# FengDushuo/BBBP-Multi-Modal-Deep-Ensemble-Framework

Measured on AMD Instinct MI355X. Metric: molecules/sec fwd+bwd (3-branch ensemble, B=512), higher is better.
Workload: dtype f32; 1 GPU; MixedInputModel F=167 (MACCS) + 3x128x128 image, 6-layer encoder + 2-stage CNN + fusion + BN head; forward + MSE + backward + fused AdamW, train mode (dropout 0.1); global_batch=512, per_gpu_batch=512, parallelism=dp1, input=device-resident

## Files before the change

bbbp-multi-modal-deep-ensemble-framework_amd/csrc/common.h:

```cpp
#pragma once
#include <hip/hip_runtime.h>
#include <stdint.h>
#include <stdio.h>
#include <string.h>

typedef float f32x16 __attribute__((ext_vector_type(16)));
typedef float f32x4 __attribute__((ext_vector_type(4)));
typedef float f32x2 __attribute__((ext_vector_type(2)));

#define BBBP_OK 0
#define BBBP_ERR_ARG 1
#define BBBP_ERR_HIP 2
#define BBBP_ERR_WORKSPACE 3

void bbbp_set_error(const char* fmt, ...);

#define BBBP_CHECK_ARG(cond, ...)                 \
    do {                                          \
        if (!(cond)) {                            \
            bbbp_set_error(__VA_ARGS__);          \
            return BBBP_ERR_ARG;                  \
        }                                         \
    } while (0)

#define BBBP_CHECK_HIP(expr)                                                            \
    do {                                                                                \
        hipError_t _e = (expr);                                                         \
        if (_e != hipSuccess) {                                                         \
            bbbp_set_error("%s failed: %s (%s:%d)", #expr, hipGetErrorString(_e), __FILE__, __LINE__); \
            return BBBP_ERR_HIP;                                                        \
        }                                                                               \
    } while (0)

#define BBBP_CHECK_LAUNCH() BBBP_CHECK_HIP(hipGetLastError())

static inline int cdiv(int a, int b) { return (a + b - 1) / b; }
static inline size_t align_up(size_t x, size_t a) { return (x + a - 1) / a * a; }

int bbbp_num_cus();
static inline int persistent_grid(int want, int nmb, int nwork) {
    int grid = want;
    if (grid >= 8 * nmb) grid -= grid % (8 * nmb);
    if (grid > nwork) grid = nwork - nwork % nmb;
    return grid < nmb ? nmb : grid;
}
int bbbp_ensure_dyn_lds(const void* kernel, size_t bytes);
template <class P>
int launch_lds(void (*kernel)(P), dim3 grid, int threads, size_t lds, hipStream_t st, const P& p) {
    if (int rc = bbbp_ensure_dyn_lds(reinterpret_cast<const void*>(kernel), lds)) return rc;
    void* args[] = {const_cast<P*>(&p)};
    BBBP_CHECK_HIP(hipLaunchKernel(reinterpret_cast<const void*>(kernel), grid, dim3(threads), args, lds, st));
    return BBBP_OK;
}
const char* bbbp_env(const char* name);
int bbbp_env_int(const char* name, int dflt);
static inline int clampi(int v, int lo, int hi) { return v < lo ? lo : (v > hi ? hi : v); }
struct Knob {
    const char* env; int dflt; int (*norm)(int);
    int v = -1;
    int get() { if (v < 0) v = norm(bbbp_env_int(env, dflt)); return v; }
    int set(int x) { const int prev = get(); v = norm(x); return prev; }
};
static inline int knob_bool(int v) { return v != 0; }

extern thread_local int g_bbbp_reserved_cus;
extern thread_local size_t g_bbbp_small_lds_pad;
struct ConvPrefs {
    int conv1_fwd_f32 = 0;
    int conv1_fwd_per_cu = 0;
    int conv2_fwd_pipe = 0;
    int wgrad_beside_encoder = 0;
};
enum ConvMaskBit {
    CONV_WINO_FWD = 1, CONV_WINO_DGRAD = 2,
    CONV_B3_FWD = 4, CONV_B3_DGRAD = 8, CONV_B3_WGRAD = 16,
    CONV_B3_C1_WGRAD = 32, CONV_B3_C1_FWD = 64,
    CONV_B3_WGRAD_SPARSE = 128, CONV_B3_WGRAD_SPARSE4 = 256,
    CONV_MASK_ALL = 511
};
enum class ConvForm { F32Direct, Winograd, SplitBf16, SplitBf16Pipe, Conv1SplitBf16, Conv1SplitBf16Pipe, WgradDense, WgradSparse8, WgradSparse4 };
int conv3x3_relu_pool_fwd(hipStream_t st, const float* x, const float* w, const float* bias, float* y, uint8_t* mask, int B, int cin, int cout,
                          int H, int W, void* workspace, size_t workspace_bytes, const ConvPrefs& prefs);
int conv3x3_relu_pool_bwd_weight(hipStream_t st, const float* x, const float* gy, const uint8_t* gmask, float* dw, float* dbias, int B, int cin,
                                 int cout, int H, int W, void* workspace, size_t workspace_bytes, const ConvPrefs& prefs);
extern thread_local int g_bbbp_wino_side_cus;
int bbbp_head_forward_fused(hipStream_t st, const float* comb, const float* const* fw1, const float* const* fb1,
                            const float* const* fw2, const float* const* fb2, const float* w0, const float* b0, const float* gamma,
                            const float* beta, float* running_mean, float* running_var, const float* w3, const float* b3,
                            const float* w5, const float* b5, const float* w7, const float* b7, float* hid, float* attn, float* fused,
                            float* h, float* hb, float* bn_mean, float* bn_rstd, float* h2, float* h3, float* out, float* partial,
                            int B, int training, int concat);
int bbbp_head_backward_fused(hipStream_t st, const float* dout, const float* comb, const float* hid, const float* attn, const float* h,
                             const float* h2, const float* h3, const float* bn_mean, const float* bn_rstd, const float* gamma,
                             const float* const* fw1, const float* const* fw2, const float* w0, const float* w3, const float* w5,
                             const float* w7, float* dh3, float* dh2, float* dhb, float* dh, float* dlogit, float* dpre, float* dcomb,
                             float* dgamma, float* dbeta, float* partial, int B, int training);
struct bbbp_enc_row_fwd_args {
    const float* ctx; const float* xin;
    const float *wo, *bo, *g1, *be1, *w1, *b1, *w2, *b2, *g2, *be2;
    const float *wn, *bn; float* outn; int nn, ldn, actn;
    float *z1, *y1, *hff, *z2, *y2, *mean1, *rstd1, *mean2, *rstd2;
    int B, F, DFF; float p; uint64_t seed1, seed2, seed3;
};
struct bbbp_enc_row_bwd_args {
    const float* dqkv_up; const float* win_up; const float* dz1_up; float* dyout;
    const float *z2, *mean2, *rstd2, *g2, *w2, *hff, *w1, *z1, *mean1, *rstd1, *g1, *wo;
    float *dz2, *dff, *dhff, *dy1, *dz1, *dsa, *dctx;
    int B, F, DFF; float p; uint64_t seed1, seed3;
};
bool bbbp_enc_rows_supported(int F, int nhead, int dff);
int bbbp_enc_row_fwd(hipStream_t st, const bbbp_enc_row_fwd_args* a);
int bbbp_enc_row_bwd(hipStream_t st, const bbbp_enc_row_bwd_args* a);
int bbbp_ln_param_grad_multi(hipStream_t st, int n, const float* const* dy, const float* const* z, const float* const* mean,
                             const float* const* rstd, float* const* dgamma, float* const* dbeta, int rows, int cols);
bool bbbp_attn_small_supported(int B, int nhead, int head_dim);
bool bbbp_attn_wide_supported(int B, int nhead, int head_dim);
size_t bbbp_attn_small_keep_bytes(int B, int nhead, int head_dim);
int bbbp_attn_small_fwd(hipStream_t st, const float* qkv, float* ctx, float* lse, int B, int F, int nhead, float scale, float p, uint64_t seed,
                        uint8_t* keep = nullptr);
int bbbp_attn_small_bwd(hipStream_t st, const float* qkv, const float* ctx, const float* lse, const float* dctx, float* dqkv, int B, int F,
                        int nhead, float scale, float p, uint64_t seed, const uint8_t* keep = nullptr);
constexpr size_t BBBP_CONV_MIN_LDS = 120 * 1024;
int bbbp_wino_conv2_fwd(hipStream_t st, const float* x, const float* w, const float* bias, float* y, uint8_t* mask, int B,
                        float* workspace);
int bbbp_wino_conv2_dgrad(hipStream_t st, const float* gy, const uint8_t* gmask, const float* w, float* dx, int B, float* workspace);
int bbbp_wino_last_clock(unsigned long long* shader_cycles, unsigned long long* ticks_100mhz);
bool bbbp_b3_conv_supported(int cin, int cout, int hw);
size_t bbbp_b3_workspace_bytes(int cin, int cout);
int bbbp_b3_conv_fwd(hipStream_t st, const float* x, const float* w, const float* bias, float* y, uint8_t* mask, int B, int cin, int cout, void* workspace,
                     ConvForm form, int per_cu, bool probe);
int bbbp_b3_conv_dgrad(hipStream_t st, const float* gy, const uint8_t* gmask, const float* w, float* dx, int B, int cin, int cout, void* workspace,
                       ConvForm form, int per_cu, bool probe);
int bbbp_b3_conv2_wgrad(hipStream_t st, const float* x, const float* gy, const uint8_t* mask, float* slab, float* bslab, int B, int grid, ConvForm form,
                        int cin_total, int cout_total, int groups, int map);
int bbbp_b3_last_clock(unsigned long long* shader_cycles, unsigned long long* ticks_100mhz);
size_t bbbp_b3_conv1_fwd_workspace_bytes();
int bbbp_b3_conv1_fwd(hipStream_t st, const float* x, const float* w, const float* bias, float* y, uint8_t* mask, int B, void* workspace,
                      ConvForm form, int per_cu);
int bbbp_b3_conv1_wgrad(hipStream_t st, const float* x, const float* gy, const uint8_t* mask, float* slab, float* bslab, int B, int grid);
int bbbp_wino_last_phases(unsigned long long* phases4);
int bbbp_param_wait(hipStream_t st, const void* ptr);
bool bbbp_param_pending_elsewhere(const void* ptr);
bool bbbp_layernorm_linear_preferred(int M, int N, int K);
bool bbbp_outproj_fold_supported(int F, int nhead, int layers);
size_t bbbp_outproj_fold_floats(int F, int which);
int bbbp_outproj_fold(hipStream_t st, int layers, int F, const float* const* win, const float* const* bin, const float* const* wo,
                      const float* const* bo, float* const* wf, float* const* bf, float* const* wvt);
int bbbp_outproj_unfold(hipStream_t st, int F, int B, const float* tdw, const float* tdb, const float* wo, const float* wvt, const float* dz,
                        int lddz, float* g_outw, float* g_outb, float* g_inw_v, float* g_inb_v);

__device__ __forceinline__ int xcd_adjacent(int w, int n) { return (n & 7) ? w : (w & 7) * (n >> 3) + (w >> 3); }

__device__ __forceinline__ f32x16 mfma32(float a, float b, f32x16 c) {
    return __builtin_amdgcn_mfma_f32_32x32x2f32(a, b, c, 0, 0, 0);
}
__device__ __forceinline__ int mfma_row(int r, int lane) { return (r & 3) + 8 * (r >> 2) + 4 * (lane >> 5); }

typedef __bf16 bf16x8 __attribute__((ext_vector_type(8)));
typedef __bf16 bf16x2 __attribute__((ext_vector_type(2)));
typedef float f32x2v __attribute__((ext_vector_type(2)));
typedef uint32_t u32x4 __attribute__((ext_vector_type(4)));
typedef uint32_t u32x2 __attribute__((ext_vector_type(2)));
__device__ __forceinline__ void split2(float a, float b, uint32_t& hi, uint32_t& mid, uint32_t& lo) {
    f32x2v v = {a, b};
    bf16x2 h = __builtin_convertvector(v, bf16x2);
    hi = __builtin_bit_cast(uint32_t, h);
    f32x2v hf = {__builtin_bit_cast(float, hi << 16), __builtin_bit_cast(float, hi & 0xffff0000u)};
    v = v - hf;
    bf16x2 m = __builtin_convertvector(v, bf16x2);
    mid = __builtin_bit_cast(uint32_t, m);
    f32x2v mf = {__builtin_bit_cast(float, mid << 16), __builtin_bit_cast(float, mid & 0xffff0000u)};
    v = v - mf;
    bf16x2 l = __builtin_convertvector(v, bf16x2);
    lo = __builtin_bit_cast(uint32_t, l);
}

__device__ __forceinline__ uint4 philox4(uint64_t seed, uint64_t ctr) {
    uint32_t k0 = (uint32_t)seed, k1 = (uint32_t)(seed >> 32);
    uint32_t c0 = (uint32_t)ctr, c1 = (uint32_t)(ctr >> 32), c2 = 0x9E3779B9u, c3 = 0xBB67AE85u;
#pragma unroll
    for (int i = 0; i < 10; ++i) {
        uint64_t p0 = (uint64_t)0xD2511F53u * c0;
        uint64_t p1 = (uint64_t)0xCD9E8D57u * c2;
        uint32_t n0 = (uint32_t)(p1 >> 32) ^ c1 ^ k0;
        uint32_t n1 = (uint32_t)p1;
        uint32_t n2 = (uint32_t)(p0 >> 32) ^ c3 ^ k1;
        uint32_t n3 = (uint32_t)p0;
        c0 = n0; c1 = n1; c2 = n2; c3 = n3;
        k0 += 0x9E3779B9u; k1 += 0xBB67AE85u;
    }
    return make_uint4(c0, c1, c2, c3);
}
extern thread_local const unsigned long long* g_bbbp_seed_base;
__device__ __forceinline__ uint64_t effective_seed(uint64_t seed, const unsigned long long* base) {
    return base ? (uint64_t)(*base) * 0x9E3779B97F4A7C15ull + seed : seed;
}
__device__ __forceinline__ float dropout_scale(uint64_t seed, uint64_t idx, float p, float inv_keep) {
    uint4 r = philox4(seed, idx >> 2);
    uint32_t v = (idx & 3) == 0 ? r.x : (idx & 3) == 1 ? r.y : (idx & 3) == 2 ? r.z : r.w;
    float u = (float)(v >> 8) * (1.0f / 16777216.0f);
    return u >= p ? inv_keep : 0.0f;
}

#ifndef BBBP_HIGH_PRIO
#define BBBP_HIGH_PRIO() __builtin_amdgcn_s_setprio(3)
#endif
```

bbbp-multi-modal-deep-ensemble-framework_amd/csrc/conv.hip:

```cpp
#include "common.h"
#include "bbbp_hip.h"
#include <limits.h>
#include <algorithm>
#include <stdlib.h>

namespace {

constexpr int MODE_FWD = 0;
constexpr int MODE_DGRAD = 1;
constexpr int PADL = 4;

struct ConvParams {
    const float* x;
    const uint8_t* xmask;
    const float* wt;
    const float* bias;
    float* y;
    uint8_t* ymask;
    int B, H;
    int co_total;
};

template <int CIN, int COUT, int W, int MODE>
struct ConvCfg {
// ... 565 lines not shown
        for (int i = 0; i < X_NIT; ++i) {
            int idx = t + i * 512;
            if (idx >= X_ITEMS) continue;
            int q = idx % (W / 4), row = (idx / (W / 4)) % 4, ci = idx / (W / 4 * 4);
            float* d = xs + ci * PLANE + row * LDW + PADL + q * 4;
            d[0] = xq[i].x; d[1] = xq[i].y; d[2] = xq[i].z; d[3] = xq[i].w;
        }
    };

    constexpr int PIX_PER_W = C::NPIX / 8;
    const int pix0 = wave * PIX_PER_W;
    const int prow = pix0 / W, pcol = pix0 % W;
    const int j = lane & 31, k2 = lane >> 5;
    const int jj = j < 27 ? j : 0;
    const int boff = (jj / 9) * PLANE + ((jj % 9) / 3) * LDW + (jj % 3);
    const int abase = j * LDP + pix0 + k2;
    const int bbase = boff + prow * LDW + pcol + k2 + PADL - 1;
    const float bsel = j < 27 ? 1.f : 0.f;

    f32x16 acc;
#pragma unroll
    for (int r = 0; r < 16; ++r) acc[r] = 0.f;

    int strip = xcd_adjacent(grp, p.groups);
    if (strip < nstrips) { load_stage(strip); store_stage(0); }
    __syncthreads();
    int buf = 0;
    for (; strip < nstrips; strip += p.groups) {
        const int nstrip = strip + p.groups;
        if (nstrip < nstrips) load_stage(nstrip);
        const float* dys = smem + buf * C::BUF + abase;
        const float* xs = smem + buf * C::BUF + C::DYF + bbase;
#pragma unroll
        for (int pp = 0; pp < PIX_PER_W; pp += 2) acc = mfma32(dys[pp], xs[pp] * bsel, acc);
        if (nstrip < nstrips) store_stage(buf ^ 1);
        __syncthreads();
        buf ^= 1;
    }
    float* red = smem;
    for (int g = 1; g < 8; ++g) {
        if (wave == g) {
#pragma unroll
            for (int r = 0; r < 16; ++r) red[r * 64 + lane] = acc[r];
        }
        __syncthreads();
        if (wave == 0) {
#pragma unroll
            for (int r = 0; r < 16; ++r) acc[r] += red[r * 64 + lane];
        }
        __syncthreads();
    }
#pragma unroll
    for (int i = 0; i < DY_NIT; ++i) {
        float v = bsum[i];
#pragma unroll
        for (int o = 1; o < Wp / 4; o <<= 1) v += __shfl_xor(v, o);
        int idx = t + i * 512;
        if (idx < DY_ITEMS && idx % (Wp / 4) == 0) p.bslab[(long)blockIdx.x * COUT + idx / (Wp / 4)] = v;
    }
    if (wave == 0) {
        float* s = p.slab + (long)blockIdx.x * 1024;
#pragma unroll
        for (int r = 0; r < 16; ++r) s[mfma_row(r, lane) * 32 + j] = acc[r];
    }
}

__global__ __launch_bounds__(1024) void conv_wgrad3_reduce_kernel(const float* slab, const float* bslab, float* dw,
                                                                 float* db, int groups) {
    __shared__ float part[32][32];
    const int cob = blockIdx.y;
    const float* sl = slab + (long)cob * groups * 1024;
    const float* bs = bslab + (long)cob * groups * 32;
    const int nl = threadIdx.x & 31, grp = threadIdx.x >> 5;
    const int n = blockIdx.x * 32 + nl;
    const int per = (groups + 31) / 32, g0 = min(groups, grp * per), g1 = min(groups, g0 + per);
    float s = 0.f;
    if (n < 1024) s = slab_sum(sl + n, 1024, g0, g1);
    else s = slab_sum(bs + (n - 1024), 32, g0, g1);
    part[grp][nl] = s;
    __syncthreads();
    if (grp == 0) {
        float v = 0.f;
#pragma unroll
        for (int i = 0; i < 32; ++i) v += part[i][nl];
        if (n < 1024) { if ((n & 31) < 27) dw[(cob * 32 + (n >> 5)) * 27 + (n & 31)] = v; }
        else db[cob * 32 + (n - 1024)] = v;
    }
}

template <int CIN, int COUT, int W, int MODE>
int launch_conv(const ConvParams& p, hipStream_t st) {
    using C = ConvCfg<CIN, COUT, W, MODE>;
    const bool part = g_bbbp_reserved_cus > 0;
    size_t lds = C::LDS_BYTES;
    if (part && lds < BBBP_CONV_MIN_LDS) lds = BBBP_CONV_MIN_LDS;
    int nstrips = p.B * (p.H / C::TH);
    int per_cu = (int)((160 * 1024) / lds);
    if (per_cu > 2) per_cu = 2;
    if (per_cu < 1) per_cu = 1;
    static const int cap = bbbp_env_int("BBBP_CONV_PER_CU", 0);
    if (cap > 0 && per_cu > cap) per_cu = cap;
    int cus = bbbp_num_cus() - (part ? g_bbbp_reserved_cus : 0);
    if (cus < 1) cus = 1;
    int grid = cus * per_cu;
    if (grid > nstrips) grid = nstrips;
    return launch_lds(conv3x3_kernel<CIN, COUT, W, MODE>, grid, C::NT, lds, st, p);
}

inline bool supported(int cin, int cout, int h, int w) {
    if (h != w) return false;
    return (cin == 3 && cout == 32 && w == 128) || (cin == 32 && cout == 64 && w == 64) || (cin == 3 && cout == 64 && w == 128) ||
           (cin == 64 && cout == 128 && w == 64) || (cin == 128 && cout == 256 && w == 32);
}

Knob g_winograd{"BBBP_CONV_WINOGRAD", 252, [](int v) { return v & CONV_MASK_ALL; }};
thread_local int g_bbbp_conv2_fwd_pipe = 0;
thread_local int g_bbbp_conv_wgrad_beside_encoder = 0;

struct ConvKnobs {
    int c2_pipe;
    int c2_dgrad_pipe;
    int b3_probe;
    int b3_per_cu;
    int wgrad_sparse_waves;
    int c1_pipe;
    int c1_per_cu;
};
const ConvKnobs& conv_knobs() {
    static const ConvKnobs k{bbbp_env_int("BBBP_C2_PIPE", INT_MIN), bbbp_env_int("BBBP_C2_DGRAD_PIPE", 0), bbbp_env_int("BBBP_B3_PROBE", 0),
                             clampi(bbbp_env_int("BBBP_B3_PER_CU", 2), 1, 2), bbbp_env_int("BBBP_C2_WGRAD_SPARSE_WAVES", 0),
                             bbbp_env_int("BBBP_C1_PIPE", 1), clampi(bbbp_env_int("BBBP_C1_PER_CU", 2), 1, 4)};
    return k;
}

enum class ConvOp { Fwd, Dgrad, Wgrad };
enum class ConvClock { Keep, F32, Winograd, SplitBf16 };
struct ConvChoice {
    ConvForm form = ConvForm::F32Direct;
    size_t workspace = 0;
    ConvClock clock = ConvClock::F32;
    int per_cu = 0;
    bool probe = false;
};
ConvClock g_last_clock = ConvClock::F32;

ConvChoice conv_choice(ConvOp op, int cin, int cout, int hw, int mask, const ConvPrefs& prefs, const ConvKnobs& kn) {
    ConvChoice c;
    const bool b3_stage = bbbp_b3_conv_supported(cin, cout, hw), conv2 = cin == 32 && cout == 64, conv1 = cin == 3 && cout == 32 && hw == 128;
    auto at_least = [&](size_t bytes) { if (c.workspace < bytes) c.workspace = bytes; };
    if (op == ConvOp::Wgrad) {
        c.workspace = (size_t)2 * 256 * (cin == 3 ? 1024 + 32 : (size_t)64 * 288 + 64) * sizeof(float);
        c.clock = ConvClock::Keep;
        const bool sparse = (mask & CONV_B3_WGRAD_SPARSE) != 0;
        if (conv1 && (mask & CONV_B3_C1_WGRAD)) c.form = ConvForm::Conv1SplitBf16;
        else if (b3_stage && (mask & CONV_B3_WGRAD) && (sparse || hw == 64)) {
            const int waves = kn.wgrad_sparse_waves ? kn.wgrad_sparse_waves : (((mask & CONV_B3_WGRAD_SPARSE4) || prefs.wgrad_beside_encoder) ? 4 : 8);
            c.form = !sparse ? ConvForm::WgradDense : waves == 8 ? ConvForm::WgradSparse8 : ConvForm::WgradSparse4;
        }
        return c;
    }
    const bool fwd = op == ConvOp::Fwd;
    c.workspace = (size_t)9 * (fwd && cin < 8 ? 4 : cin) * cout * sizeof(float);
    if (b3_stage && (mask & (fwd ? CONV_B3_FWD : CONV_B3_DGRAD))) {
        const int pipe = !fwd ? kn.c2_dgrad_pipe : kn.c2_pipe != INT_MIN ? kn.c2_pipe : prefs.conv2_fwd_pipe;
        c.form = (hw == 64 && pipe && !kn.b3_probe) ? ConvForm::SplitBf16Pipe : ConvForm::SplitBf16;
        c.per_cu = kn.b3_per_cu; c.probe = kn.b3_probe != 0;
        c.clock = ConvClock::SplitBf16;
        at_least(bbbp_b3_workspace_bytes(cin, cout));
    } else if (conv2 && (mask & (fwd ? CONV_WINO_FWD : CONV_WINO_DGRAD))) {
        c.form = ConvForm::Winograd;
        c.clock = ConvClock::Winograd;
        at_least((size_t)16 * 32 * 64 * sizeof(float));
    } else if (fwd && conv1 && (mask & CONV_B3_C1_FWD) && !prefs.conv1_fwd_f32) {
        c.form = kn.c1_pipe ? ConvForm::Conv1SplitBf16Pipe : ConvForm::Conv1SplitBf16;
        c.per_cu = prefs.conv1_fwd_per_cu > 0 ? prefs.conv1_fwd_per_cu : kn.c1_per_cu;
        at_least(bbbp_b3_conv1_fwd_workspace_bytes());
    }
    return c;
}
ConvChoice conv_choice(ConvOp op, int cin, int cout, int hw, const ConvPrefs& prefs) { return conv_choice(op, cin, cout, hw, g_winograd.get(), prefs, conv_knobs()); }

}

extern "C" int bbbp_set_conv_winograd(int mask) {
    BBBP_CHECK_ARG(mask >= 0 && mask <= CONV_MASK_ALL, "set_conv_winograd: mask %d (bits 0/1 Winograd forward / data gradient, bits 2/3/4 split-bf16 forward / data gradient / weight gradient of conv2, bits 5/6 split-bf16 weight gradient / forward of conv1, bit 7 conv2's split-bf16 weight gradient on the structured-sparse MFMA, bit 8 its 4-wave form)", mask);
    g_winograd.set(mask);
    return BBBP_OK;
}

extern "C" int bbbp_get_conv_winograd(void) { return g_winograd.get(); }
extern "C" int bbbp_conv_winograd_phases(unsigned long long* phases4) {
    BBBP_CHECK_ARG(phases4, "conv_winograd_phases: null pointer");
    return bbbp_wino_last_phases(phases4);
}

extern "C" int bbbp_conv_last_clock(unsigned long long* shader_cycles, unsigned long long* ticks_100mhz) {
    BBBP_CHECK_ARG(shader_cycles && ticks_100mhz, "conv_last_clock: null pointer");
    if (g_last_clock == ConvClock::SplitBf16) return bbbp_b3_last_clock(shader_cycles, ticks_100mhz);
    if (g_last_clock == ConvClock::Winograd) return bbbp_wino_last_clock(shader_cycles, ticks_100mhz);
    unsigned long long h[2] = {0, 0};
    BBBP_CHECK_HIP(hipMemcpyFromSymbol(h, HIP_SYMBOL(g_conv_clock), sizeof(h)));
    *shader_cycles = h[0]; *ticks_100mhz = h[1];
    return BBBP_OK;
}

extern "C" size_t bbbp_conv3x3_workspace_bytes(int B, int cin, int cout, int H, int W) {
    (void)B; (void)W;
    auto need = [&](ConvOp op) { return conv_choice(op, cin, cout, H, ConvPrefs{}).workspace; };
    return align_up(std::max({need(ConvOp::Fwd), need(ConvOp::Dgrad), need(ConvOp::Wgrad)}), 256);
}

extern "C" int bbbp_set_conv_wgrad_beside_encoder(int on) {
    const int prev = g_bbbp_conv_wgrad_beside_encoder;
    g_bbbp_conv_wgrad_beside_encoder = on ? 1 : 0;
    return prev;
}
extern "C" int bbbp_set_conv2_fwd_pipe(int on) {
    const int prev = g_bbbp_conv2_fwd_pipe;
    g_bbbp_conv2_fwd_pipe = on ? 1 : 0;
    return prev;
}

extern "C" int bbbp_conv3x3_relu_pool_fwd(void* stream, const float* x, const float* w, const float* bias,
                                          float* y, uint8_t* mask, int B, int cin, int cout, int H, int W,
                                          void* workspace, size_t workspace_bytes) {
    ConvPrefs prefs;
    prefs.conv2_fwd_pipe = g_bbbp_conv2_fwd_pipe;
    return conv3x3_relu_pool_fwd(static_cast<hipStream_t>(stream), x, w, bias, y, mask, B, cin, cout, H, W, workspace, workspace_bytes, prefs);
}

int conv3x3_relu_pool_fwd(hipStream_t st, const float* x, const float* w, const float* bias, float* y, uint8_t* mask, int B, int cin, int cout,
                          int H, int W, void* workspace, size_t workspace_bytes, const ConvPrefs& prefs) {
    BBBP_CHECK_ARG(supported(cin, cout, H, W), "conv fwd: unsupported shape cin=%d cout=%d H=%d W=%d", cin, cout, H, W);
    BBBP_CHECK_ARG(x && w && bias && y && workspace, "conv fwd: null pointer");
    if (B == 0) return BBBP_OK;
    const ConvChoice c = conv_choice(ConvOp::Fwd, cin, cout, H, prefs);
    BBBP_CHECK_ARG(workspace_bytes >= c.workspace, "conv fwd: workspace %zu < %zu", workspace_bytes, c.workspace);
    float* wt = static_cast<float*>(workspace);
    g_last_clock = c.clock;
    if (c.form == ConvForm::SplitBf16 || c.form == ConvForm::SplitBf16Pipe)
        return bbbp_b3_conv_fwd(st, x, w, bias, y, mask, B, cin, cout, workspace, c.form, c.per_cu, c.probe);
    if (c.form == ConvForm::Winograd) return bbbp_wino_conv2_fwd(st, x, w, bias, y, mask, B, wt);
    if (c.form != ConvForm::F32Direct) return bbbp_b3_conv1_fwd(st, x, w, bias, y, mask, B, workspace, c.form, c.per_cu);
    const int cinp = cin < 8 ? 4 : cin, total = 9 * cinp * cout;
    hipLaunchKernelGGL(conv_prep_weights_kernel, dim3(cdiv(total, 256)), dim3(256), 0, st, w, wt, cin, cout, cinp, MODE_FWD);
    BBBP_CHECK_LAUNCH();
    ConvParams p{x, nullptr, wt, bias, y, mask, B, H, cout};
    if (cin == 3 && cout == 32) return launch_conv<3, 32, 128, MODE_FWD>(p, st);
    if (cin == 3 && cout == 64) return launch_conv<3, 64, 128, MODE_FWD>(p, st);
    if (cin == 32) return launch_conv<32, 64, 64, MODE_FWD>(p, st);
    if (cin == 64) return launch_conv<64, 64, 64, MODE_FWD>(p, st);
    return launch_conv<128, 64, 32, MODE_FWD>(p, st);
}

extern "C" int bbbp_conv3x3_relu_pool_bwd_data(void* stream, const float* gy, const uint8_t* mask, const float* w,
                                               float* dx, int B, int cin, int cout, int H, int W,
                                               void* workspace, size_t workspace_bytes) {
    BBBP_CHECK_ARG(supported(cin, cout, H, W) && cin != 3,
                   "conv bwd_data: unsupported shape cin=%d cout=%d H=%d W=%d", cin, cout, H, W);
    BBBP_CHECK_ARG(gy && mask && w && dx && workspace, "conv bwd_data: null pointer");
    if (B == 0) return BBBP_OK;
    hipStream_t st = static_cast<hipStream_t>(stream);
    const ConvChoice c = conv_choice(ConvOp::Dgrad, cin, cout, H, ConvPrefs{});
    BBBP_CHECK_ARG(workspace_bytes >= c.workspace, "conv bwd_data: workspace %zu < %zu", workspace_bytes, c.workspace);
    float* wt = static_cast<float*>(workspace);
    g_last_clock = c.clock;
    if (c.form == ConvForm::SplitBf16 || c.form == ConvForm::SplitBf16Pipe)
        return bbbp_b3_conv_dgrad(st, gy, mask, w, dx, B, cin, cout, workspace, c.form, c.per_cu, c.probe);
    if (c.form == ConvForm::Winograd) return bbbp_wino_conv2_dgrad(st, gy, mask, w, dx, B, wt);
    int total = 9 * cout * cin;
    hipLaunchKernelGGL(conv_prep_weights_kernel, dim3(cdiv(total, 256)), dim3(256), 0, st, w, wt, cin, cout, 0, MODE_DGRAD);
    BBBP_CHECK_LAUNCH();
    ConvParams p{gy, mask, wt, nullptr, dx, nullptr, B, H, cin};
    if (cin == 32) return launch_conv<64, 32, 64, MODE_DGRAD>(p, st);
    if (cin == 64) return launch_conv<128, 64, 64, MODE_DGRAD>(p, st);
    return launch_conv<256, 64, 32, MODE_DGRAD>(p, st);
}

template <int W, int CIN_TOTAL, int COUT_TOTAL>
static int launch_wgrad32(WgradParams p, int grid, hipStream_t st) {
    return launch_lds(conv_wgrad32_kernel<64, W, CIN_TOTAL, COUT_TOTAL>, grid, 512, WgCfg<64, W>::LDS_BYTES, st, p);
}

extern "C" int bbbp_conv3x3_relu_pool_bwd_weight(void* stream, const float* x, const float* gy, const uint8_t* mask,
                                                 float* dw, float* db, int B, int cin, int cout, int H, int W,
                                                 void* workspace, size_t workspace_bytes) {
    ConvPrefs prefs;
    prefs.wgrad_beside_encoder = g_bbbp_conv_wgrad_beside_encoder;
    return conv3x3_relu_pool_bwd_weight(static_cast<hipStream_t>(stream), x, gy, mask, dw, db, B, cin, cout, H, W, workspace, workspace_bytes, prefs);
}

int conv3x3_relu_pool_bwd_weight(hipStream_t st, const float* x, const float* gy, const uint8_t* mask, float* dw, float* db, int B, int cin,
                                 int cout, int H, int W, void* workspace, size_t workspace_bytes, const ConvPrefs& prefs) {
    BBBP_CHECK_ARG(supported(cin, cout, H, W), "conv bwd_weight: unsupported shape cin=%d cout=%d H=%d W=%d", cin, cout, H, W);
    BBBP_CHECK_ARG(x && gy && mask && dw && db && workspace, "conv bwd_weight: null pointer");
    if (B == 0) {
        BBBP_CHECK_HIP(hipMemsetAsync(dw, 0, (size_t)cout * cin * 9 * sizeof(float), st));
        BBBP_CHECK_HIP(hipMemsetAsync(db, 0, (size_t)cout * sizeof(float), st));
        return BBBP_OK;
    }
    const ConvChoice c = conv_choice(ConvOp::Wgrad, cin, cout, H, prefs);
    int nstrips = B * (H / 2);
    const bool part = g_bbbp_reserved_cus > 0;
    const int ncu = bbbp_num_cus(), cus = ncu - (part ? g_bbbp_reserved_cus : 0) > 0 ? ncu - (part ? g_bbbp_reserved_cus : 0) : 1;
    float* slab = static_cast<float*>(workspace);
    WgradParams p{x, gy, mask, slab, nullptr, B, H, cin, cout, 1};
    if (cin == 3) {
        using C = Wg3Cfg<128>;
        const int ncob = cout / 32;
        size_t lds3 = C::LDS_BYTES;
        if (part) lds3 = BBBP_CONV_MIN_LDS;
        const int groups = clampi((part ? cus : ncu * 2) / ncob, 1, nstrips);
        const int grid = groups * ncob;
        BBBP_CHECK_ARG(workspace_bytes >= (size_t)grid * (1024 + 32) * sizeof(float), "conv bwd_weight: workspace too small");
        p.groups = groups;
        p.bslab = slab + (size_t)grid * 1024;
        const int rc = c.form == ConvForm::Conv1SplitBf16 ? bbbp_b3_conv1_wgrad(st, x, gy, mask, slab, p.bslab, B, grid)
                                                          : launch_lds(conv_wgrad3_kernel<128>, grid, 512, lds3, st, p);
        if (rc) return rc;
        hipLaunchKernelGGL(conv_wgrad3_reduce_kernel, dim3(33, ncob), dim3(1024), 0, st, slab, p.bslab, dw, db, groups);
        BBBP_CHECK_LAUNCH();
    } else {
        const int pairs = (cin / 32) * (cout / 64);
        const int groups = clampi(cus / pairs, 1, nstrips);
        const int grid = groups * pairs;
        BBBP_CHECK_ARG(workspace_bytes >= (size_t)grid * (64 * 288 + 64) * sizeof(float), "conv bwd_weight: workspace too small");
        p.groups = groups;
        p.bslab = slab + (size_t)grid * 64 * 288;
        int rc;
        if (c.form != ConvForm::F32Direct) rc = bbbp_b3_conv2_wgrad(st, x, gy, mask, slab, p.bslab, B, grid, c.form, cin, cout, groups, W);
        else rc = cin == 32 ? launch_wgrad32<64, 32, 64>(p, grid, st)
               : cin == 64 ? launch_wgrad32<64, 64, 128>(p, grid, st) : launch_wgrad32<32, 128, 256>(p, grid, st);
        if (rc) return rc;
        hipLaunchKernelGGL(conv_wgrad32_reduce_kernel, dim3(cdiv(64 * 289, 64), pairs), dim3(1024), 0, st, slab, p.bslab, dw, db,
                           groups, cin, cout);
        BBBP_CHECK_LAUNCH();
    }
    return BBBP_OK;
}
```

bbbp-multi-modal-deep-ensemble-framework_amd/csrc/conv_b3.hip:

```cpp
#include "common.h"
#include "bbbp_hip.h"

namespace {

constexpr int B3_FWD = 0, B3_DGRAD = 1;
constexpr int IMG = 64;
constexpr int R = 4, ROWS = R + 2;
constexpr int PXW = IMG + 2;
constexpr int CH = 16;
constexpr int XPLANE = ROWS * PXW * CH;
constexpr int XBUF = 3 * XPLANE;
constexpr int WSTAGE = 9 * 3 * 2 * 32 * 8;
[[maybe_unused]] constexpr size_t LDS_BYTES = (size_t)(XBUF + WSTAGE) * 2;

struct B3Params {
    const float* x;
    const uint8_t* xmask;
    const uint16_t* wp;
    const float* bias;
    float* y;
    uint8_t* ymask;
    int B;
    int prio;
};
// ... 889 lines not shown
    const uint8_t* mask;
    float* slab;
    float* bslab;
    int B;
    int prio;
};

__global__ __launch_bounds__(256) void conv_b3_wgrad3_kernel(B3Wgrad3Params p) {
    if (p.prio >= 3) __builtin_amdgcn_s_setprio(3); else if (p.prio == 2) __builtin_amdgcn_s_setprio(2); else if (p.prio == 1) __builtin_amdgcn_s_setprio(1);
    extern __shared__ __attribute__((aligned(16))) uint16_t smem[];
    uint16_t* DYs = smem;
    uint16_t* X1s = smem + 3 * DY1PLANE;
    const int t = threadIdx.x, lane = t & 63, wave = t >> 6, r = lane & 31, h = lane >> 5;
    const int nstrips = p.B * (IMG1 / 2);
    for (int i = t * 8; i < 3 * DY1PLANE + 3 * X1PLANE; i += 256 * 8) *reinterpret_cast<u32x4*>(smem + i) = u32x4{0, 0, 0, 0};

    f32x4 gq[2][2]; uint32_t mq[2][2]; f32x4 xq[2][2];
    uint32_t okx[2] = {0, 0};
    float bsum[2] = {0.f, 0.f};
    const int xi_q = t & 15, xi_row = (t >> 4) & 3, xi_ci = min(t >> 6, 2);
    auto load_stage = [&](int strip, int set) __attribute__((always_inline)) {
        const int b = strip / (IMG1 / 2), ph = strip % (IMG1 / 2);
#pragma unroll
        for (int i = 0; i < 2; ++i) {
            const int idx = t + i * 256, q = idx & 15, co = idx >> 4;
            const long off = (((long)b * 32 + co) * (IMG1 / 2) + ph) * (IMG1 / 2) + q * 4;
            gq[set][i] = *reinterpret_cast<const f32x4*>(p.gy + off);
            mq[set][i] = *reinterpret_cast<const uint32_t*>(p.mask + off);
        }
        const int yr = 2 * ph - 1 + xi_row;
        okx[set] = (yr >= 0 && yr < IMG1 && t < 192) ? 1u : 0u;
        const float* src = p.x + (((long)b * 3 + xi_ci) * IMG1 + min(max(yr, 0), IMG1 - 1)) * IMG1 + xi_q * 8;
        xq[set][0] = *reinterpret_cast<const f32x4*>(src);
        xq[set][1] = *reinterpret_cast<const f32x4*>(src + 4);
    };
    auto store_stage = [&](int set) __attribute__((always_inline)) {
#pragma unroll
        for (int i = 0; i < 2; ++i) {
            const int idx = t + i * 256, q = idx & 15, co = idx >> 4;
            float v0[8], v1[8];
#pragma unroll
            for (int e = 0; e < 4; ++e) {
                const uint32_t m = (mq[set][i] >> (8 * e)) & 0xff;
                const float g = gq[set][i][e];
                bsum[i] += m < 4 ? g : 0.f;
                v0[2 * e] = m == 0 ? g : 0.f; v0[2 * e + 1] = m == 1 ? g : 0.f;
                v1[2 * e] = m == 2 ? g : 0.f; v1[2 * e + 1] = m == 3 ? g : 0.f;
            }
            uint32_t hi[4], mid[4], lo[4];
            uint16_t* d = DYs + co * DY1CO + q * 8;
#pragma unroll
            for (int j = 0; j < 4; ++j) split2(v0[2 * j], v0[2 * j + 1], hi[j], mid[j], lo[j]);
            *reinterpret_cast<u32x4*>(d) = u32x4{hi[0], hi[1], hi[2], hi[3]};
            *reinterpret_cast<u32x4*>(d + DY1PLANE) = u32x4{mid[0], mid[1], mid[2], mid[3]};
            *reinterpret_cast<u32x4*>(d + 2 * DY1PLANE) = u32x4{lo[0], lo[1], lo[2], lo[3]};
#pragma unroll
            for (int j = 0; j < 4; ++j) split2(v1[2 * j], v1[2 * j + 1], hi[j], mid[j], lo[j]);
            *reinterpret_cast<u32x4*>(d + IMG1) = u32x4{hi[0], hi[1], hi[2], hi[3]};
            *reinterpret_cast<u32x4*>(d + IMG1 + DY1PLANE) = u32x4{mid[0], mid[1], mid[2], mid[3]};
            *reinterpret_cast<u32x4*>(d + IMG1 + 2 * DY1PLANE) = u32x4{lo[0], lo[1], lo[2], lo[3]};
        }
        if (t < 192) {
            const bool ok = okx[set] != 0;
            uint32_t hi[4], mid[4], lo[4];
#pragma unroll
            for (int j = 0; j < 4; ++j) {
                const float a = j < 2 ? xq[set][0][2 * j] : xq[set][1][2 * j - 4], c = j < 2 ? xq[set][0][2 * j + 1] : xq[set][1][2 * j - 3];
                split2(ok ? a : 0.f, ok ? c : 0.f, hi[j], mid[j], lo[j]);
            }
            uint16_t* d = X1s + xi_ci * X1CI + xi_row * X1ROW + 8 + xi_q * 8;
            *reinterpret_cast<u32x4*>(d) = u32x4{hi[0], hi[1], hi[2], hi[3]};
            *reinterpret_cast<u32x4*>(d + X1PLANE) = u32x4{mid[0], mid[1], mid[2], mid[3]};
            *reinterpret_cast<u32x4*>(d + 2 * X1PLANE) = u32x4{lo[0], lo[1], lo[2], lo[3]};
        }
    };

    f32x16 acc;
#pragma unroll
    for (int q = 0; q < 16; ++q) acc[q] = 0.f;
    const int jj = r < 27 ? r : 0;
    const int ci = jj / 9, kh = (jj % 9) / 3, kw = jj % 3;
    const uint16_t* abase = DYs + r * DY1CO + 8 * h;
    const uint16_t* bbase = X1s + ci * X1CI + kh * X1ROW + 8 + 8 * h;
    const uint32_t shift = kw == 1 ? 0u : 16u;

    const int stride = gridDim.x;
    int strip = xcd_adjacent(blockIdx.x, gridDim.x);
    __syncthreads();
    if (strip < nstrips) { load_stage(strip, 0); store_stage(0); }
    if (strip + stride < nstrips) load_stage(strip + stride, 1);
    for (; strip < nstrips; strip += 2 * stride) {
#pragma unroll
        for (int u = 0; u < 2; ++u) {
            const int cur = strip + u * stride;
            if (cur >= nstrips) break;
            __syncthreads();
            if (cur + 2 * stride < nstrips) load_stage(cur + 2 * stride, u);
#pragma unroll
            for (int s4 = 0; s4 < 4; ++s4) {
                const int ks = wave * 4 + s4, rr = ks >> 3, x0 = (ks & 7) * 16;
                bf16x8 a[3], bf[3];
#pragma unroll
                for (int pl = 0; pl < 3; ++pl) {
                    a[pl] = *reinterpret_cast<const bf16x8*>(abase + pl * DY1PLANE + rr * IMG1 + x0);
                    const uint16_t* src = bbase + pl * X1PLANE + rr * X1ROW + x0;
                    const u32x4 w = *reinterpret_cast<const u32x4*>(src);
                    const uint32_t wm = *reinterpret_cast<const uint32_t*>(src - 2), wp = *reinterpret_cast<const uint32_t*>(src + 8);
                    const uint32_t l0 = kw == 0 ? wm : w[0], l1 = kw == 0 ? w[0] : w[1], l2 = kw == 0 ? w[1] : w[2], l3 = kw == 0 ? w[2] : w[3];
                    const uint32_t u0 = kw == 0 ? w[0] : w[1], u1 = kw == 0 ? w[1] : w[2], u2 = kw == 0 ? w[2] : w[3], u3 = kw == 0 ? w[3] : wp;
                    const uint32_t c0 = kw == 1 ? w[0] : l0, c1 = kw == 1 ? w[1] : l1, c2 = kw == 1 ? w[2] : l2, c3 = kw == 1 ? w[3] : l3;
                    const u32x4 f = {__builtin_amdgcn_alignbit(u0, c0, shift), __builtin_amdgcn_alignbit(u1, c1, shift),
                                     __builtin_amdgcn_alignbit(u2, c2, shift), __builtin_amdgcn_alignbit(u3, c3, shift)};
                    bf[pl] = __builtin_bit_cast(bf16x8, f);
                }
                acc = __builtin_amdgcn_mfma_f32_32x32x16_bf16(a[1], bf[1], acc, 0, 0, 0);
                acc = __builtin_amdgcn_mfma_f32_32x32x16_bf16(a[2], bf[0], acc, 0, 0, 0);
                acc = __builtin_amdgcn_mfma_f32_32x32x16_bf16(a[0], bf[2], acc, 0, 0, 0);
                acc = __builtin_amdgcn_mfma_f32_32x32x16_bf16(a[1], bf[0], acc, 0, 0, 0);
                acc = __builtin_amdgcn_mfma_f32_32x32x16_bf16(a[0], bf[1], acc, 0, 0, 0);
                acc = __builtin_amdgcn_mfma_f32_32x32x16_bf16(a[0], bf[0], acc, 0, 0, 0);
            }
            __syncthreads();
            if (cur + stride < nstrips) store_stage(u ^ 1);
        }
    }
    __syncthreads();
    float* red = reinterpret_cast<float*>(smem);
    for (int g = 1; g < 4; ++g) {
        if (wave == g) {
#pragma unroll
            for (int q = 0; q < 16; ++q) red[q * 64 + lane] = acc[q];
        }
        __syncthreads();
        if (wave == 0) {
#pragma unroll
            for (int q = 0; q < 16; ++q) acc[q] += red[q * 64 + lane];
        }
        __syncthreads();
    }
    if (wave == 0) {
        float* sdst = p.slab + (long)blockIdx.x * 1024;
#pragma unroll
        for (int q = 0; q < 16; ++q) sdst[mfma_row(q, lane) * 32 + r] = acc[q];
    }
#pragma unroll
    for (int i = 0; i < 2; ++i) {
        float v = bsum[i];
        v += __shfl_xor(v, 1); v += __shfl_xor(v, 2); v += __shfl_xor(v, 4); v += __shfl_xor(v, 8);
        const int idx = t + i * 256;
        if ((idx & 15) == 0) p.bslab[(long)blockIdx.x * 32 + (idx >> 4)] = v;
    }
}

template <int MODE, class G>
int launch_b3(const B3Params& p, hipStream_t st, ConvForm form, int per_cu, bool probe) {
    constexpr bool flagship = G::CIN == 32 && G::COUT == 64 && G::IMGS == 64;
    constexpr int IMGL = G::IMGS, RL = 256 / IMGL, NMB = (MODE == B3_FWD ? G::COUT : G::CIN) / 32;
    constexpr size_t lds = (size_t)(3 * (RL + 2) * (IMGL + 2) * CH + WSTAGE) * 2;
    const int nwork = p.B * (IMGL / RL) * NMB;
    if constexpr (G::IMGS == 64) {
        if (form == ConvForm::SplitBf16Pipe) {
            auto pk = MODE == B3_FWD ? (p.ymask ? conv_b3p_kernel<MODE, G, true> : conv_b3p_kernel<MODE, G, false>) : conv_b3p_kernel<MODE, G, false>;
            return launch_lds(pk, persistent_grid(bbbp_num_cus(), NMB, nwork), 256, 2 * lds, st, p);
        }
    }
    auto kernel = conv_b3_kernel<MODE, G>;
    if constexpr (flagship) { if (probe) kernel = conv_b3_probe_kernel<MODE>; }
    return launch_lds(kernel, persistent_grid(bbbp_num_cus() * per_cu, NMB, nwork), 256, lds, st, p);
}

template <int MODE>
int launch_b3_stage(const B3Params& p, int cin, hipStream_t st, ConvForm form, int per_cu, bool probe) {
    if (cin == 32) return launch_b3<MODE, GeomFlagship>(p, st, form, per_cu, probe);
    if (cin == 64) return launch_b3<MODE, B3Geom<64, 128, 64>>(p, st, form, per_cu, probe);
    return launch_b3<MODE, B3Geom<128, 256, 32>>(p, st, form, per_cu, probe);
}

}

bool bbbp_b3_conv_supported(int cin, int cout, int hw) {
    return (cin == 32 && cout == 64 && hw == 64) || (cin == 64 && cout == 128 && hw == 64) || (cin == 128 && cout == 256 && hw == 32);
}
size_t bbbp_b3_workspace_bytes(int cin, int cout) {
    const size_t fwd = (size_t)(cin / 16) * (cout / 32) * WSTAGE * 2, dgrad = (size_t)(cout / 16) * (cin / 32) * WSTAGE * 2;
    return fwd > dgrad ? fwd : dgrad;
}

static int conv_bwd_prio() {
    static const int v = clampi(bbbp_env_int("BBBP_CONV_BWD_PRIO", 0), 0, 3);
    return v;
}

int bbbp_b3_conv_fwd(hipStream_t st, const float* x, const float* w, const float* bias, float* y, uint8_t* mask, int B, int cin, int cout, void* workspace,
                     ConvForm form, int per_cu, bool probe) {
    hipLaunchKernelGGL(b3_prep_kernel, dim3(cin * cout >= 64 * 128 ? 288 : 72), dim3(256), 0, st, w, static_cast<uint16_t*>(workspace), B3_FWD, cin, cout);
    BBBP_CHECK_LAUNCH();
    B3Params p{x, nullptr, static_cast<const uint16_t*>(workspace), bias, y, mask, B, 0};
    return launch_b3_stage<B3_FWD>(p, cin, st, form, per_cu, probe);
}

int bbbp_b3_conv_dgrad(hipStream_t st, const float* gy, const uint8_t* gmask, const float* w, float* dx, int B, int cin, int cout, void* workspace,
                       ConvForm form, int per_cu, bool probe) {
    hipLaunchKernelGGL(b3_prep_kernel, dim3(cin * cout >= 64 * 128 ? 288 : 72), dim3(256), 0, st, w, static_cast<uint16_t*>(workspace), B3_DGRAD, cin, cout);
    BBBP_CHECK_LAUNCH();
    B3Params p{gy, gmask, static_cast<const uint16_t*>(workspace), nullptr, dx, nullptr, B, conv_bwd_prio()};
    return launch_b3_stage<B3_DGRAD>(p, cin, st, form, per_cu, probe);
}

extern "C" int bbbp_conv_b3_phases(unsigned long long* phases4) {
    BBBP_CHECK_ARG(phases4, "conv_b3_phases: null pointer");
    BBBP_CHECK_HIP(hipMemcpyFromSymbol(phases4, HIP_SYMBOL(g_b3_phase), 4 * sizeof(unsigned long long)));
    return BBBP_OK;
}

int bbbp_b3_conv2_wgrad(hipStream_t st, const float* x, const float* gy, const uint8_t* mask, float* slab, float* bslab, int B, int grid, ConvForm form,
                        int cin_total, int cout_total, int groups, int map) {
    B3WgradParams p{x, gy, mask, slab, bslab, B, conv_bwd_prio(), cin_total, cout_total, groups};
    const bool dense = form == ConvForm::WgradDense, w8 = form == ConvForm::WgradSparse8;
    BBBP_CHECK_ARG(dense || w8 || form == ConvForm::WgradSparse4, "b3 weight gradient: not a weight-gradient form (%d)", (int)form);
    BBBP_CHECK_ARG(map == 64 || (map == 32 && !dense), "b3 weight gradient: 64 x 64 maps (any form) or 32 x 32 maps (structured-sparse forms), got %d / form %d", map, (int)form);
    if (dense) return launch_lds(conv_b3_wgrad_kernel, grid, 256, (size_t)WG_LDS_BYTES, st, p);
    if (map == 32) return w8 ? launch_lds(conv_b3_wgrad_sp_kernel<8, 32>, grid, 512, WGS_LDS_BYTES, st, p)
                             : launch_lds(conv_b3_wgrad_sp_kernel<4, 32>, grid, 256, WGS_LDS_BYTES, st, p);
    return w8 ? launch_lds(conv_b3_wgrad_sp_kernel<8>, grid, 512, WGS_LDS_BYTES, st, p) : launch_lds(conv_b3_wgrad_sp_kernel<4>, grid, 256, WGS_LDS_BYTES, st, p);
}

int bbbp_b3_conv1_wgrad(hipStream_t st, const float* x, const float* gy, const uint8_t* mask, float* slab, float* bslab, int B, int grid) {
    B3Wgrad3Params p{x, gy, mask, slab, bslab, B, conv_bwd_prio()};
    return launch_lds(conv_b3_wgrad3_kernel, grid, 256, (size_t)WG3_LDS_BYTES, st, p);
}

int bbbp_b3_last_clock(unsigned long long* shader_cycles, unsigned long long* ticks_100mhz) {
    unsigned long long h[2] = {0, 0};
    BBBP_CHECK_HIP(hipMemcpyFromSymbol(h, HIP_SYMBOL(g_b3_clock), sizeof(h)));
    *shader_cycles = h[0]; *ticks_100mhz = h[1];
    return BBBP_OK;
}
```

Before: 223,800 molecules/s.

## Add compact split-bf16 conv1 weight-gradient kernel with LDS-side mask expansion

Adds a new conv1 weight-gradient kernel that stores pooled gradients compactly in LDS with per-element byte-select words, expanding them to the unpooled layout via v_perm at MFMA time. It also pre-shifts the input rows for the three kw taps using DPP and alignbit into rotated LDS slots, and double-buffers strip loads in registers. The smaller LDS footprint is sized for two work-groups per CU. The previous kernel stays selectable through a new mask bit; the new kernel becomes the default whenever the conv1 split-bf16 weight gradient is enabled.

```diff
diff --git a/bbbp-multi-modal-deep-ensemble-framework_amd/csrc/common.h b/bbbp-multi-modal-deep-ensemble-framework_amd/csrc/common.h
--- a/bbbp-multi-modal-deep-ensemble-framework_amd/csrc/common.h
+++ b/bbbp-multi-modal-deep-ensemble-framework_amd/csrc/common.h
@@ -76,9 +76,10 @@
     CONV_B3_FWD = 4, CONV_B3_DGRAD = 8, CONV_B3_WGRAD = 16,
     CONV_B3_C1_WGRAD = 32, CONV_B3_C1_FWD = 64,
     CONV_B3_WGRAD_SPARSE = 128, CONV_B3_WGRAD_SPARSE4 = 256,
-    CONV_MASK_ALL = 511
-};
-enum class ConvForm { F32Direct, Winograd, SplitBf16, SplitBf16Pipe, Conv1SplitBf16, Conv1SplitBf16Pipe, WgradDense, WgradSparse8, WgradSparse4 };
+    CONV_B3_C1_WGRAD_PRE = 512,
+    CONV_MASK_ALL = 1023
+};
+enum class ConvForm { F32Direct, Winograd, SplitBf16, SplitBf16Pipe, Conv1SplitBf16, Conv1SplitBf16Pipe, WgradDense, WgradSparse8, WgradSparse4, Conv1SplitBf16Pre };
 int conv3x3_relu_pool_fwd(hipStream_t st, const float* x, const float* w, const float* bias, float* y, uint8_t* mask, int B, int cin, int cout,
                           int H, int W, void* workspace, size_t workspace_bytes, const ConvPrefs& prefs);
 int conv3x3_relu_pool_bwd_weight(hipStream_t st, const float* x, const float* gy, const uint8_t* gmask, float* dw, float* dbias, int B, int cin,
@@ -137,7 +138,7 @@
 size_t bbbp_b3_conv1_fwd_workspace_bytes();
 int bbbp_b3_conv1_fwd(hipStream_t st, const float* x, const float* w, const float* bias, float* y, uint8_t* mask, int B, void* workspace,
                       ConvForm form, int per_cu);
-int bbbp_b3_conv1_wgrad(hipStream_t st, const float* x, const float* gy, const uint8_t* mask, float* slab, float* bslab, int B, int grid);
+int bbbp_b3_conv1_wgrad(hipStream_t st, const float* x, const float* gy, const uint8_t* mask, float* slab, float* bslab, int B, int grid, ConvForm form);
 int bbbp_wino_last_phases(unsigned long long* phases4);
 int bbbp_param_wait(hipStream_t st, const void* ptr);
 bool bbbp_param_pending_elsewhere(const void* ptr);
diff --git a/bbbp-multi-modal-deep-ensemble-framework_amd/csrc/conv.hip b/bbbp-multi-modal-deep-ensemble-framework_amd/csrc/conv.hip
--- a/bbbp-multi-modal-deep-ensemble-framework_amd/csrc/conv.hip
+++ b/bbbp-multi-modal-deep-ensemble-framework_amd/csrc/conv.hip
@@ -741,7 +741,7 @@
         c.workspace = (size_t)2 * 256 * (cin == 3 ? 1024 + 32 : (size_t)64 * 288 + 64) * sizeof(float);
         c.clock = ConvClock::Keep;
         const bool sparse = (mask & CONV_B3_WGRAD_SPARSE) != 0;
-        if (conv1 && (mask & CONV_B3_C1_WGRAD)) c.form = ConvForm::Conv1SplitBf16;
+        if (conv1 && (mask & CONV_B3_C1_WGRAD)) c.form = (mask & CONV_B3_C1_WGRAD_PRE) ? ConvForm::Conv1SplitBf16Pre : ConvForm::Conv1SplitBf16;
         else if (b3_stage && (mask & CONV_B3_WGRAD) && (sparse || hw == 64)) {
             const int waves = kn.wgrad_sparse_waves ? kn.wgrad_sparse_waves : (((mask & CONV_B3_WGRAD_SPARSE4) || prefs.wgrad_beside_encoder) ? 4 : 8);
             c.form = !sparse ? ConvForm::WgradDense : waves == 8 ? ConvForm::WgradSparse8 : ConvForm::WgradSparse4;
@@ -772,7 +772,7 @@
 }
 
 extern "C" int bbbp_set_conv_winograd(int mask) {
-    BBBP_CHECK_ARG(mask >= 0 && mask <= CONV_MASK_ALL, "set_conv_winograd: mask %d (bits 0/1 Winograd forward / data gradient, bits 2/3/4 split-bf16 forward / data gradient / weight gradient of conv2, bits 5/6 split-bf16 weight gradient / forward of conv1, bit 7 conv2's split-bf16 weight gradient on the structured-sparse MFMA, bit 8 its 4-wave form)", mask);
+    BBBP_CHECK_ARG(mask >= 0 && mask <= CONV_MASK_ALL, "set_conv_winograd: mask %d (bits 0/1 Winograd forward / data gradient, bits 2/3/4 split-bf16 forward / data gradient / weight gradient of conv2, bits 5/6 split-bf16 weight gradient / forward of conv1, bit 7 conv2's split-bf16 weight gradient on the structured-sparse MFMA, bit 8 its 4-wave form, bit 9 conv1's split-bf16 weight gradient in its earlier form)", mask);
     g_winograd.set(mask);
     return BBBP_OK;
 }
@@ -904,7 +904,7 @@
         BBBP_CHECK_ARG(workspace_bytes >= (size_t)grid * (1024 + 32) * sizeof(float), "conv bwd_weight: workspace too small");
         p.groups = groups;
         p.bslab = slab + (size_t)grid * 1024;
-        const int rc = c.form == ConvForm::Conv1SplitBf16 ? bbbp_b3_conv1_wgrad(st, x, gy, mask, slab, p.bslab, B, grid)
+        const int rc = c.form != ConvForm::F32Direct ? bbbp_b3_conv1_wgrad(st, x, gy, mask, slab, p.bslab, B, grid, c.form)
                                                           : launch_lds(conv_wgrad3_kernel<128>, grid, 512, lds3, st, p);
         if (rc) return rc;
         hipLaunchKernelGGL(conv_wgrad3_reduce_kernel, dim3(33, ncob), dim3(1024), 0, st, slab, p.bslab, dw, db, groups);
diff --git a/bbbp-multi-modal-deep-ensemble-framework_amd/csrc/conv_b3.hip b/bbbp-multi-modal-deep-ensemble-framework_amd/csrc/conv_b3.hip
--- a/bbbp-multi-modal-deep-ensemble-framework_amd/csrc/conv_b3.hip
+++ b/bbbp-multi-modal-deep-ensemble-framework_amd/csrc/conv_b3.hip
@@ -1065,6 +1065,179 @@
     }
 }
 
+constexpr int P1CO = IMG1 / 2 + 4;
+constexpr int P1PLANE = 32 * P1CO;
+constexpr int S1CO = 2 * 16 * 4 + 4;
+constexpr int X1IMG = 4 * IMG1;
+constexpr int X1SPLANE = 9 * X1IMG;
+constexpr size_t WG3S_LDS_BYTES = (size_t)(3 * P1PLANE + 3 * X1SPLANE) * 2 + (size_t)32 * S1CO * 4;
+static_assert(2 * WG3S_LDS_BYTES <= 160 * 1024, "two work-groups per CU");
+constexpr uint64_t X1ROT = 0x9F802C3C6ull;
+__device__ __forceinline__ int x1rot(int kw, int ci) { return (int)(X1ROT >> (4 * (kw * 3 + ci))) & 15; }
+
+__global__ __launch_bounds__(256) void conv_b3_wgrad3s_kernel(B3Wgrad3Params p) {
+    if (p.prio >= 3) __builtin_amdgcn_s_setprio(3); else if (p.prio == 2) __builtin_amdgcn_s_setprio(2); else if (p.prio == 1) __builtin_amdgcn_s_setprio(1);
+    extern __shared__ __attribute__((aligned(16))) uint16_t smem[];
+    uint16_t* Ps = smem;
+    uint32_t* Ss = reinterpret_cast<uint32_t*>(smem + 3 * P1PLANE);
+    uint16_t* X1s = smem + 3 * P1PLANE + 2 * 32 * S1CO;
+    const int t = threadIdx.x, lane = t & 63, wave = t >> 6, r = lane & 31, h = lane >> 5;
+    const int nstrips = p.B * (IMG1 / 2);
+
+    f32x4 gq[2][2]; uint32_t mq[2][2]; f32x4 xq[2][2];
+    uint32_t okx[2] = {0, 0};
+    float bsum[2] = {0.f, 0.f};
+    const int xi_q = t & 15, xi_row = (t >> 4) & 3, xi_ci = min(t >> 6, 2);
+    auto load_stage = [&](int strip, int set) __attribute__((always_inline)) {
+        const int b = strip / (IMG1 / 2), ph = strip % (IMG1 / 2);
+#pragma unroll
+        for (int i = 0; i < 2; ++i) {
+            const int idx = t + i * 256, q = idx & 15, co = idx >> 4;
+            const long off = (((long)b * 32 + co) * (IMG1 / 2) + ph) * (IMG1 / 2) + q * 4;
+            gq[set][i] = *reinterpret_cast<const f32x4*>(p.gy + off);
+            mq[set][i] = *reinterpret_cast<const uint32_t*>(p.mask + off);
+        }
+        const int yr = 2 * ph - 1 + xi_row;
+        okx[set] = (yr >= 0 && yr < IMG1 && t < 192) ? 1u : 0u;
+        const float* src = p.x + (((long)b * 3 + xi_ci) * IMG1 + min(max(yr, 0), IMG1 - 1)) * IMG1 + xi_q * 8;
+        xq[set][0] = *reinterpret_cast<const f32x4*>(src);
+        xq[set][1] = *reinterpret_cast<const f32x4*>(src + 4);
+    };
+    uint16_t* xdst[3];
+#pragma unroll
+    for (int kw = 0; kw < 3; ++kw)
+        xdst[kw] = X1s + (kw * 3 + xi_ci) * X1IMG + xi_row * IMG1 + ((xi_q + x1rot(kw, xi_ci) + xi_row) & 15) * 8;
+    auto store_stage = [&](int set) __attribute__((always_inline)) {
+#pragma unroll
+        for (int i = 0; i < 2; ++i) {
+            const int idx = t + i * 256, q = idx & 15, co = idx >> 4;
+            uint32_t pc[2][3];
+            split2(gq[set][i][0], gq[set][i][1], pc[0][0], pc[0][1], pc[0][2]);
+            split2(gq[set][i][2], gq[set][i][3], pc[1][0], pc[1][1], pc[1][2]);
+            u32x4 sel[2];
+#pragma unroll
+            for (int e = 0; e < 4; ++e) {
+                const uint32_t m = (mq[set][i] >> (8 * e)) & 0xff;
+                bsum[i] += m < 4 ? gq[set][i][e] : 0.f;
+                const uint32_t from = (e & 1) ? 0x0302u : 0x0100u, even = 0x0c0c0000u | from, odd = (from << 16) | 0x0c0cu, none = 0x0c0c0c0cu;
+                sel[0][e] = m == 0 ? even : m == 1 ? odd : none;
+                sel[1][e] = m == 2 ? even : m == 3 ? odd : none;
+            }
+#pragma unroll
+            for (int pl = 0; pl < 3; ++pl) *reinterpret_cast<u32x2*>(Ps + pl * P1PLANE + co * P1CO + q * 4) = u32x2{pc[0][pl], pc[1][pl]};
+            *reinterpret_cast<u32x4*>(Ss + co * S1CO + q * 4) = sel[0];
+            *reinterpret_cast<u32x4*>(Ss + co * S1CO + 64 + q * 4) = sel[1];
+        }
+        if (t < 192) {
+            const bool ok = okx[set] != 0;
+            uint32_t pcx[3][4];
+#pragma unroll
+            for (int j = 0; j < 4; ++j) {
+                const float a = j < 2 ? xq[set][0][2 * j] : xq[set][1][2 * j - 4], c = j < 2 ? xq[set][0][2 * j + 1] : xq[set][1][2 * j - 3];
+                split2(ok ? a : 0.f, ok ? c : 0.f, pcx[0][j], pcx[1][j], pcx[2][j]);
+            }
+#pragma unroll
+            for (int pl = 0; pl < 3; ++pl) {
+                const uint32_t* w = pcx[pl];
+                const uint32_t left = (uint32_t)__builtin_amdgcn_update_dpp(0, (int)w[3], 0x111, 0xF, 0xF, false);
+                const uint32_t right = (uint32_t)__builtin_amdgcn_update_dpp(0, (int)w[0], 0x101, 0xF, 0xF, false);
+                const uint32_t m01 = __builtin_amdgcn_alignbit(w[1], w[0], 16), m12 = __builtin_amdgcn_alignbit(w[2], w[1], 16),
+                               m23 = __builtin_amdgcn_alignbit(w[3], w[2], 16);
+                *reinterpret_cast<u32x4*>(xdst[0] + pl * X1SPLANE) = u32x4{__builtin_amdgcn_alignbit(w[0], left, 16), m01, m12, m23};
+                *reinterpret_cast<u32x4*>(xdst[1] + pl * X1SPLANE) = u32x4{w[0], w[1], w[2], w[3]};
+                *reinterpret_cast<u32x4*>(xdst[2] + pl * X1SPLANE) = u32x4{m01, m12, m23, __builtin_amdgcn_alignbit(right, w[3], 16)};
+            }
+        }
+    };
+
+    f32x16 acc;
+#pragma unroll
+    for (int q = 0; q < 16; ++q) acc[q] = 0.f;
+    const int jj = r < 27 ? r : 0;
+    const int ci = jj / 9, kh = (jj % 9) / 3, kw = jj % 3;
+    const int rr = wave >> 1;
+    const int item0 = (wave & 1) * 8 + h;
+    const uint16_t* abase = Ps + r * P1CO + item0 * 4;
+    const uint32_t* sbase = Ss + r * S1CO + rr * 64 + item0 * 4;
+    const uint16_t* bbase = X1s + (kw * 3 + ci) * X1IMG + (kh + rr) * IMG1;
+    const int bslot = (wave & 1) * 8 + h + x1rot(kw, ci) + kh + rr;
+    int boff[4];
+#pragma unroll
+    for (int s4 = 0; s4 < 4; ++s4) boff[s4] = ((bslot + 2 * s4) & 15) * 8;
+    struct Frag { u32x2 pc[3]; u32x4 sel; bf16x8 bf[3]; };
+    auto fetch = [&](int s4, Frag& f) __attribute__((always_inline)) {
+        f.sel = *reinterpret_cast<const u32x4*>(sbase + s4 * 8);
+#pragma unroll
+        for (int pl = 0; pl < 3; ++pl) {
+            f.pc[pl] = *reinterpret_cast<const u32x2*>(abase + pl * P1PLANE + s4 * 8);
+            f.bf[pl] = *reinterpret_cast<const bf16x8*>(bbase + pl * X1SPLANE + boff[s4]);
+        }
+    };
+    auto expand = [&](const Frag& f, int pl) __attribute__((always_inline)) {
+        const u32x4 w = {__builtin_amdgcn_perm(f.pc[pl][0], f.pc[pl][0], f.sel[0]), __builtin_amdgcn_perm(f.pc[pl][0], f.pc[pl][0], f.sel[1]),
+                         __builtin_amdgcn_perm(f.pc[pl][1], f.pc[pl][1], f.sel[2]), __builtin_amdgcn_perm(f.pc[pl][1], f.pc[pl][1], f.sel[3])};
+        return __builtin_bit_cast(bf16x8, w);
+    };
+
+    const int stride = gridDim.x;
+    int strip = xcd_adjacent(blockIdx.x, gridDim.x);
+    if (strip < nstrips) { load_stage(strip, 0); store_stage(0); }
+    if (strip + stride < nstrips) load_stage(strip + stride, 1);
+    for (; strip < nstrips; strip += 2 * stride) {
+#pragma unroll
+        for (int u = 0; u < 2; ++u) {
+            const int cur = strip + u * stride;
+            if (cur >= nstrips) break;
+            __syncthreads();
+            if (cur + 2 * stride < nstrips) load_stage(cur + 2 * stride, u);
+            Frag fr[2];
+            fetch(0, fr[0]);
+            __builtin_amdgcn_sched_barrier(0);
+#pragma unroll
+            for (int s4 = 0; s4 < 4; ++s4) {
+                const Frag& f = fr[s4 & 1];
+                if (s4 < 3) fetch(s4 + 1, fr[(s4 & 1) ^ 1]);
+                __builtin_amdgcn_sched_barrier(0);
+                const bf16x8 a1 = expand(f, 1), a2 = expand(f, 2), a0 = expand(f, 0);
+                acc = __builtin_amdgcn_mfma_f32_32x32x16_bf16(a1, f.bf[1], acc, 0, 0, 0);
+                acc = __builtin_amdgcn_mfma_f32_32x32x16_bf16(a2, f.bf[0], acc, 0, 0, 0);
+                acc = __builtin_amdgcn_mfma_f32_32x32x16_bf16(a0, f.bf[2], acc, 0, 0, 0);
+                acc = __builtin_amdgcn_mfma_f32_32x32x16_bf16(a1, f.bf[0], acc, 0, 0, 0);
+                acc = __builtin_amdgcn_mfma_f32_32x32x16_bf16(a0, f.bf[1], acc, 0, 0, 0);
+                acc = __builtin_amdgcn_mfma_f32_32x32x16_bf16(a0, f.bf[0], acc, 0, 0, 0);
+            }
+            __syncthreads();
+            if (cur + stride < nstrips) store_stage(u ^ 1);
+        }
+    }
+    __syncthreads();
+    float* red = reinterpret_cast<float*>(smem);
+    for (int g = 1; g < 4; ++g) {
+        if (wave == g) {
+#pragma unroll
+            for (int q = 0; q < 16; ++q) red[q * 64 + lane] = acc[q];
+        }
+        __syncthreads();
+        if (wave == 0) {
+#pragma unroll
+            for (int q = 0; q < 16; ++q) acc[q] += red[q * 64 + lane];
+        }
+        __syncthreads();
+    }
+    if (wave == 0) {
+        float* sdst = p.slab + (long)blockIdx.x * 1024;
+#pragma unroll
+        for (int q = 0; q < 16; ++q) sdst[mfma_row(q, lane) * 32 + r] = acc[q];
+    }
+#pragma unroll
+    for (int i = 0; i < 2; ++i) {
+        float v = bsum[i];
+        v += __shfl_xor(v, 1); v += __shfl_xor(v, 2); v += __shfl_xor(v, 4); v += __shfl_xor(v, 8);
+        const int idx = t + i * 256;
+        if ((idx & 15) == 0) p.bslab[(long)blockIdx.x * 32 + (idx >> 4)] = v;
+    }
+}
+
 template <int MODE, class G>
 int launch_b3(const B3Params& p, hipStream_t st, ConvForm form, int per_cu, bool probe) {
     constexpr bool flagship = G::CIN == 32 && G::COUT == 64 && G::IMGS == 64;
@@ -1138,9 +1311,11 @@
     return w8 ? launch_lds(conv_b3_wgrad_sp_kernel<8>, grid, 512, WGS_LDS_BYTES, st, p) : launch_lds(conv_b3_wgrad_sp_kernel<4>, grid, 256, WGS_LDS_BYTES, st, p);
 }
 
-int bbbp_b3_conv1_wgrad(hipStream_t st, const float* x, const float* gy, const uint8_t* mask, float* slab, float* bslab, int B, int grid) {
+int bbbp_b3_conv1_wgrad(hipStream_t st, const float* x, const float* gy, const uint8_t* mask, float* slab, float* bslab, int B, int grid, ConvForm form) {
     B3Wgrad3Params p{x, gy, mask, slab, bslab, B, conv_bwd_prio()};
-    return launch_lds(conv_b3_wgrad3_kernel, grid, 256, (size_t)WG3_LDS_BYTES, st, p);
+    BBBP_CHECK_ARG(form == ConvForm::Conv1SplitBf16 || form == ConvForm::Conv1SplitBf16Pre, "b3 conv1 weight gradient: not one of its forms (%d)", (int)form);
+    if (form == ConvForm::Conv1SplitBf16Pre) return launch_lds(conv_b3_wgrad3_kernel, grid, 256, (size_t)WG3_LDS_BYTES, st, p);
+    return launch_lds(conv_b3_wgrad3s_kernel, grid, 256, WG3S_LDS_BYTES, st, p);
 }
 
 int bbbp_b3_last_clock(unsigned long long* shader_cycles, unsigned long long* ticks_100mhz) {
```

After: 224,000 molecules/s, median of 5. No clear change (+0.1%).
